# millecker/hadoop-1.0.3-gpu

Hardware: AMD Instinct MI355X
Metric: K-Means job makespan + map-tasks/sec (whole node) at 1/2/4/8 MI355X (higher is better)
Workload: dtype fp32

## Files before the change

### hbmr/models/kmeans.py

```python
from __future__ import annotations

import base64
import logging
import math
import os
import threading
import time

import numpy as np
import torch

from ..gpu.splitjob import SplitJob, SplitSpec
from ..mapred import counters as C

log = logging.getLogger("hbmr.kmeans")

K_KEY = "hbmr.kmeans.k"
D_KEY = "hbmr.kmeans.dims"
INPUT_KEY = "hbmr.kmeans.input"
SPLIT_PTS_KEY = "hbmr.split.points"
CIN_KEY = "hbmr.kmeans.centroids.in"
COUT_KEY = "hbmr.kmeans.centroids.out"
INIT_KEY = "hbmr.kmeans.centroids.init"
NCENTERS_KEY = "hbmr.kmeans.synthetic.centers"
RETURN_KEY = "hbmr.kmeans.return.centroids"
CDIR_KEY = "hbmr.kmeans.centroids.dir"
EXACT_KEY = "hbmr.kmeans.exact"
EXACT_MFMA_KEY = "hbmr.kmeans.exact.mfma"
COMBINER_KEY = "hbmr.kmeans.combiner"
BOUNDS_KEY = "hbmr.kmeans.exact.bounds"

_M32 = 0xFFFFFFFF


def _mix32(x: torch.Tensor) -> torch.Tensor:
    x = x & _M32
    x = ((x ^ (x >> 16)) * 0x45D9F3B) & _M32
    x = ((x ^ (x >> 16)) * 0x45D9F3B) & _M32
    return x ^ (x >> 16)


def _uniform(c: torch.Tensor) -> torch.Tensor:
    return (_mix32(c).to(torch.float64) + 0.5) * (1.0 / 4294967296.0)


def _gauss(c1: torch.Tensor, c2: torch.Tensor) -> torch.Tensor:
    u1 = _uniform(c1)
    u2 = _uniform(c2)
    return torch.sqrt(-2.0 * torch.log(u1)) * torch.cos(2.0 * math.pi * u2)


def synthetic_points(seed: int, start: int, n: int, d: int, centers: int, device,
                     chunk: int = 1 << 18) -> torch.Tensor:
# ... 128 lines not shown
            g[2] += 1
            g[3].append((s, c))
        else:
            loose.append((s, c))
    parts_s, parts_c = [], []
    for bs, bc, n, members in groups.values():
        if n == bs.shape[0] and len({m[0].data_ptr() for m in members}) == n:
            parts_s.append(bs.sum(0))
            parts_c.append(bc.sum(0))
        else:
            loose.extend(members)
    if loose:
        parts_s.append(torch.stack([s for s, _ in loose]).sum(0))
        parts_c.append(torch.stack([c for _, c in loose]).sum(0))
    sums, counts = parts_s[0], parts_c[0]
    for s, c in zip(parts_s[1:], parts_c[1:]):
        sums = sums + s
        counts = counts + c
    return sums, counts


_EXACT_COUNTERS = {"stats": ("EXACT_FLAGGED_POINTS", "EXACT_RELABELLED_POINTS",
                             "EXACT_NEIGHBOUR_SCANS"),
                   "skipped": ("EXACT_BOUND_SKIPPED_POINTS",)}
_EXACT_DEVICE: dict = {}
_EXACT_LOCK = threading.Lock()


def _exact_counter(kind, cin, device):
    key = (kind, cin, str(device))
    with _EXACT_LOCK:
        t = _EXACT_DEVICE.get(key)
        if t is None:
            t = _EXACT_DEVICE[key] = torch.zeros(len(_EXACT_COUNTERS[kind]), dtype=torch.int64,
                                                 device=device)
        return t


def _pop_exact_counters(cin, device):
    got = ((names, _EXACT_DEVICE.pop((kind, cin, str(device)), None))
           for kind, names in _EXACT_COUNTERS.items())
    return [(names, t) for names, t in got if t is not None]

_BASELINES: "dict" = {}
_BASE_LOCK = threading.Lock()
_BASE_MAX = 4096

# ... 96 lines not shown
                    if _BASELINES.get(key) is b:
                        _BASELINES.pop(key)


class KMeansSplitJob(SplitJob):
    collective_reduce = True
    needs_reduce = True

    def configure(self, conf):
        self.conf = conf
        self.k = conf.get_int(K_KEY, 64)
        self.d = conf.get_int(D_KEY, 128)
        self.input = conf.get(INPUT_KEY, "synthetic:100000:1")
        self.split_points = conf.get_int(SPLIT_PTS_KEY, 500_000)
        self.cin = conf.get(CIN_KEY)
        self.cout = conf.get(COUT_KEY)
        self.centers = conf.get_int(NCENTERS_KEY, self.k)
        self.fx_shift = conf.get_int("hbmr.kmeans.fx.shift", 24)
        self.cdir = conf.get(CDIR_KEY)
        self.exact = conf.get_boolean(EXACT_KEY, False)
        self.exact_dtype = torch.bfloat16 if (conf.get(EXACT_MFMA_KEY) or "f16").lower() in (
            "bf16", "bfloat16") else torch.float16
        self.bounds = conf.get_boolean(BOUNDS_KEY, True)
        self.combiner = (conf.get(COMBINER_KEY) or "delta").lower()
        if self.combiner not in ("delta", "sorted"):
            raise ValueError(f"{COMBINER_KEY} must be delta or sorted, not {self.combiner!r}")
        init = conf.get(INIT_KEY)
        if init and self.cin and STORE.host_centroids(self.cin) is None:
            STORE.put_host(self.cin, decode_centroids(init))
        if self.cin and self.cdir and STORE.host_centroids(self.cin) is None:
            path = _centroid_file(self.cdir, self.cin)
            if os.path.exists(path):
                STORE.put_host(self.cin, torch.from_numpy(np.load(path)))

    _split_memo: dict = {}

    def get_splits(self, conf, trackers):
        if self.input.startswith("synthetic:"):
            mk = (self.input, self.split_points, self.d, self.centers, tuple(trackers),
                  self.exact)
            got = KMeansSplitJob._split_memo.get(mk)
            if got is not None:
                return got
            if len(KMeansSplitJob._split_memo) > 16:
                KMeansSplitJob._split_memo.clear()
            out = KMeansSplitJob._split_memo[mk] = self._synthetic_splits(trackers)
# ... 154 lines not shown
                off = 0
                for i in mb.new:
                    n = datas[i].shape[0]
                    mb.install(i, gall[off:off + n])
                    off += n
        return mb.finish()

    def _map_exact(self, ctxs, datas, img, delta):
        from ..ops import kmeans as km
        from ..utils.trace import TRACE
        if TRACE.on:
            TRACE.instant("kmeans.map_exact", n=len(datas))
        ctx = ctxs[0]
        scratch = self._stream_scratch(ctx, "kmeans-exact")
        stats = _exact_counter("stats", self.cin, ctx.device)
        mb = _MapBatch(ctxs, datas, self.k, img, True, delta)
        grown = None
        if mb.have:
            xs = [datas[i] for i in mb.have]
            total = sum(x.shape[0] for x in xs)
            lab = km.scratch_buf(scratch, "labcat", total, torch.int32, ctx.device)
            dws = km.scratch_buf(scratch, "dws", km.delta_workspace_bytes(total, len(xs), self.k),
                                 torch.uint8, ctx.device)
            bounds = skipped = None
            bounded = self.bounds and delta and km.bounds_supported(img)
            if bounded:
                nogap = [b for b in mb.bases if b.gap is None]
                bounds, skipped = mb.bases, _exact_counter("skipped", self.cin, ctx.device)
            km.assign_exact_batch(xs, img, stats, lab, scratch, stream=ctx.stream, bounds=bounds,
                                  skipped=skipped)
            if bounded:
                grown = {id(b): b.gap.numel() * b.gap.element_size() for b in nogap}
            km.delta_combine([x.x32 for x in xs], lab, self.k, *mb.delta_slabs(), dws, mb.bases,
                             fx_shift=img.fx_shift, stream=ctx.stream, keep_bounds=bounded)
            mb.advanced()
        for i in mb.new + mb.plain:
            s, c = mb.out[i]
            s.zero_()
            c.zero_()
            lab = km.map_split_exact(datas[i], img, s, c, scratch, stats, stream=ctx.stream)
            if i in mb.new:
                mb.install(i, lab.clone())
        return mb.finish(grown)

    def map_cpu(self, ctx, points):
        from ..ops import kmeans as km
        cen = STORE.host_centroids(self.cin)
        if cen is None:
            raise KeyError(f"centroids {self.cin!r} not resident")
        sums, counts = km.new_partials(self.k, self.d, "cpu")
        st = [0]
        km.map_split_cpu(points, cen, sums, counts, nthreads=ctx.cpu_threads,
                         fx_shift=self.fx_shift, exact=self.exact, stats=st)
# ... 360 lines not shown
```

### hbmr/ops/_lib.py

```python
from __future__ import annotations

import ctypes
import os
import threading
from pathlib import Path

import torch

_LIB_PATH = Path(__file__).resolve().parent.parent / "lib" / "libhbmr.so"
_lock = threading.Lock()
_lib = None

c_void_p = ctypes.c_void_p
c_long = ctypes.c_long
c_int = ctypes.c_int
c_uint = ctypes.c_uint
c_uint64 = ctypes.c_uint64
c_double_p = ctypes.POINTER(ctypes.c_double)

_SIGS = {
    "hbmr_kmeans_assign_bf16": (c_int, [c_void_p, c_long, c_int, c_void_p, c_void_p, c_int,
                                        c_void_p, c_void_p, c_void_p]),
    "hbmr_kmeans_accum_bf16": (c_int, [c_void_p, c_long, c_int, c_void_p, c_int, c_void_p,
                                       c_void_p, c_int, c_void_p, c_long, c_int, c_void_p]),
    "hbmr_kmeans_accum_f32": (c_int, [c_void_p, c_long, c_int, c_void_p, c_int, c_void_p,
                                      c_void_p, c_int, c_void_p, c_long, c_int, c_void_p]),
    "hbmr_kmeans_assign_top3_bf16": (c_int, [c_void_p, c_long, c_int, c_void_p, c_void_p, c_int,
                                             c_void_p, c_void_p, c_void_p, c_void_p, c_void_p]),
    "hbmr_kmeans_assign_top3_f16": (c_int, [c_void_p, c_long, c_int, c_void_p, c_void_p, c_int,
                                            c_void_p, c_void_p, c_void_p, c_void_p, c_void_p]),
    "hbmr_kmeans_exact_prep": (c_int, [c_void_p, c_long, c_int, c_int, c_int, c_int, c_void_p,
                                       c_void_p, c_void_p, c_void_p, c_void_p]),
    "hbmr_kmeans_assign_top3_q1_grouped": (c_int, [c_int, c_void_p, c_void_p, c_int, c_int,
                                                   c_void_p, c_void_p, c_void_p, c_int, c_void_p,
                                                   c_void_p, c_void_p, c_void_p, c_int, c_int,
                                                   c_void_p, c_void_p, c_void_p, c_void_p,
                                                   c_void_p, c_long, c_void_p, c_void_p]),
    "hbmr_kmeans_bound_workspace_bytes": (c_long, [c_long, c_int, c_int]),
    "hbmr_kmeans_assign_top3_q1_bounded": (c_int, [c_int, c_void_p, c_void_p, c_int, c_int,
                                                   c_void_p, c_void_p, c_int, c_void_p,
                                                   c_void_p, c_void_p, c_void_p, c_int, c_int,
                                                   c_void_p, c_void_p, c_void_p, c_void_p,
                                                   c_void_p, c_long, c_void_p,
                                                   c_void_p, c_void_p, c_void_p, c_void_p,
                                                   c_void_p, c_long, c_void_p, c_void_p]),
    "hbmr_kmeans_centroid_nbr": (c_int, [c_void_p, c_int, c_int, c_int, c_void_p, c_void_p,
                                         c_void_p, c_void_p]),
    "hbmr_kmeans_image16": (c_int, [c_void_p, c_int, c_int, c_int, c_int, c_int, c_void_p,
                                    c_void_p, c_void_p, c_void_p, c_void_p, c_void_p]),
    "hbmr_kmeans_image16_tiled": (c_int, [c_void_p, c_int, c_int, c_void_p, c_void_p]),
    "hbmr_kmeans_set_exact_kernel": (c_int, [c_int]),
    "hbmr_kmeans_get_exact_kernel": (c_int, []),
    "hbmr_kmeans_refine_f32": (c_int, [c_void_p, c_long, c_int, c_int, c_void_p, c_void_p,
                                       c_void_p, c_void_p, c_int, c_int, c_void_p, c_void_p,
                                       c_void_p, c_void_p, c_void_p, c_void_p, c_int, c_void_p,
                                       c_void_p, c_void_p, c_void_p, c_void_p, c_int,
                                       c_void_p]),
    "hbmr_kmeans_refine_batch_bytes": (c_long, [c_int, c_void_p]),
    "hbmr_kmeans_assign_top3_grouped": (c_int, [c_int, c_void_p, c_void_p, c_int, c_int,
                                                c_void_p, c_void_p, c_int, c_void_p, c_void_p,
                                                c_void_p, c_void_p, c_void_p]),
    "hbmr_kmeans_refine_batch_q1g": (c_int, [c_int, c_void_p, c_int, c_int, c_int, c_void_p,
                                             c_void_p, c_void_p, c_void_p, c_void_p, c_void_p,
                                             c_void_p, c_void_p, c_void_p, c_void_p, c_void_p,
                                             c_void_p, c_long, c_void_p, c_void_p]),
    "hbmr_kmeans_refine_batch_q1": (c_int, [c_int, c_void_p, c_int, c_int, c_int, c_int,
                                            c_void_p, c_void_p, c_void_p, c_void_p, c_void_p,
                                            c_void_p, c_void_p, c_void_p, c_void_p, c_void_p,
# ... 229 lines not shown
```

### hbmr/ops/kmeans.py

```python
from __future__ import annotations

import contextlib
import ctypes
import os
import threading

import torch

from . import _lib
from ._lib import ptr
from ..utils.trace import TRACE

SUPPORTED_DP = (64, 128, 256)
FX_SHIFT = 24
NBR_L = 256


def padded_dim(d: int) -> int:
    for dp in SUPPORTED_DP:
        if d <= dp:
            return dp
    raise ValueError(f"feature dim {d} > {SUPPORTED_DP[-1]} not supported by the MFMA kernel")


# ... 407 lines not shown
    _check_refine_dim(img)
    n = split.shape[0]
    dev = split.xb.device
    scratch = {} if scratch is None else scratch
    bufs = scratch.get(("exact", n))
    if bufs is None:
        bufs = scratch[("exact", n)] = tuple(
            torch.empty(m * n, dtype=t, device=dev)
            for m, t in ((1, torch.int32), (2, torch.int32), (1, torch.float32),
                         (2, torch.float32)))
    lab, cand, sc, mg = bufs
    assign_top3(split.xb, img, lab, cand, sc, mg, stream=stream)
    refine_f32(split, img, lab, cand, sc, mg, stats, stream=stream, scratch=scratch)
    return lab


def bounds_supported(img: CentroidImage) -> bool:
    return REFINE_VERSION >= 3 and img.dp <= 128 and GROUPED_EXACT and FUSED_Q1 and \
        img.cen.is_cuda and _lib.load().hbmr_kmeans_get_exact_kernel() == 3


def assign_exact_batch(splits: list, img: CentroidImage, stats: torch.Tensor, out: torch.Tensor,
                       scratch: dict | None = None, stream=None, bounds: list | None = None,
                       skipped: torch.Tensor | None = None) -> None:
    if not splits:
        return
    _check_refine_dim(img)
    if bounds is not None and (len(bounds) != len(splits) or not bounds_supported(img)):
        raise ValueError("bounds: one baseline per split, grouped fused v3 assign (dp <= 128)")
    dev = splits[0].xb.device
    total = sum(sp.shape[0] for sp in splits)
    if out.dtype != torch.int32 or out.numel() < total or not out.is_contiguous():
        raise ValueError("out must be contiguous int32 with room for every split's labels")
    _check_stats(stats)
    dt = splits[0].xb.dtype
    _check_rows([sp.xb for sp in splits], img.dp, (torch.bfloat16, torch.float16))
    if not all(sp.x32.is_contiguous() for sp in splits):
        raise ValueError("exact splits must hold contiguous fp32 rows")
    scratch = {} if scratch is None else scratch
    cand, sc, mg = _top3_scratch(scratch, "exact-batch", max(sp.shape[0] for sp in splits), dev)
    grouped = REFINE_VERSION >= 3 and img.dp <= 128 and GROUPED_EXACT
    with _on(stream):
        c16, ch, *norms = img.image16(dt)
        nbr = (None, None, 0) if grouped else img.neighbors()
        newref = None
        if bounds is not None:
            img.cen.record_stream(torch.cuda.current_stream())
            newref = img.cen.clone()
    lib = _lib.load()
    top3 = lib.hbmr_kmeans_assign_top3_f16 if dt == torch.float16 else \
        lib.hbmr_kmeans_assign_top3_bf16
    st = _lib.stream_handle(stream)
    pc, ps, pm = ptr(cand), ptr(sc), ptr(mg)
    base, off = out.data_ptr(), 0
    for g0 in range(0, len(splits), MAX_REFINE_BATCH):
        group = splits[g0:g0 + MAX_REFINE_BATCH]
        rb = _RefineBatch(group, img, stats, scratch, stream, c16, ch) \
            if REFINE_VERSION >= 3 else None
        if grouped:
            _exact_group(rb, base + 4 * off,
                         None if bounds is None else bounds[g0:g0 + MAX_REFINE_BATCH],
                         skipped, newref)
            off += rb.N
            continue
        if rb is not None:
            rb.open()
        for i, sp in enumerate(group):
            n = sp.shape[0]
            pl = base + 4 * off
            rc = top3(ptr(sp.xb), n, img.dp, ptr(c16), ptr(ch), img.k_pad, pl, pc, ps, pm, st)
            _lib.check(rc, "hbmr_kmeans_assign_top3")
            if rb is not None:
                rb.q1(i, pl, cand, sc, mg)
            else:
                _refine_single(lib, sp, img, norms, nbr, pl, pc, ps, pm, stats, st)
            off += n
        if rb is not None:
            rb.finish()


def order_after(bases: list, attrs: tuple, st) -> None:
    events, blocks = {}, {}
    for b in bases:
        if b.event is not None and b.stream is not None and b.stream != st:
            events[id(b.event)] = b.event
        for a in attrs:
            t = getattr(b, a)
            if t is not None:
                base = t._base if t._base is not None else t
                blocks[id(base)] = base
    for ev in events.values():
        st.wait_event(ev)
    for t in blocks.values():
        t.record_stream(st)


def _bounded_group(rb: _RefineBatch, bases, labels_ptr: int, skipped, newref):
    img, lib = rb.img, rb.lib
    cur = torch.cuda.current_stream() if rb.stream is None else rb.stream
    with torch.cuda.stream(cur):
        for b in bases:
            if b.gap is None:
                b.gap, b.ref = torch.empty(b.g.numel(), dtype=torch.float32, device=rb.dev), None
        for b, n in zip(bases, rb.sizes):
            if b.g.numel() != n or b.gap.numel() != n or \
                    (b.ref is not None and (tuple(b.ref.shape) != tuple(img.cen.shape) or
                                            not b.ref.is_contiguous())):
                raise ValueError("bounds: baseline does not match its split / the centroids")
        order_after(bases, ("g", "gap", "ref"), cur)
        need = int(lib.hbmr_kmeans_bound_workspace_bytes(rb.N, rb.B, img.k))
        bws = scratch_buf(rb.scratch, "bound_ws", need, torch.uint8, rb.dev)
    P = ctypes.c_void_p * rb.B
    cn, cmax, ce, cemax = rb.norms
    refs = [b.ref for b in bases]
    for b in bases:
        b.ref = b.pending = None
    rc = lib.hbmr_kmeans_assign_top3_q1_bounded(
        rb.B, rb.xb, rb.ns, img.dp, int(rb.dt == torch.float16), ptr(img.image16_tiled(rb.dt)),
        ptr(rb.ch), img.k_pad, labels_ptr, rb.xnorm, rb.xbn2, rb.xerr, img.d, img.k, ptr(cn),
        ptr(cmax), ptr(ce), ptr(cemax), ptr(rb.ws), rb.ws.numel(), ptr(rb.pd),
        P(*[b.g.data_ptr() for b in bases]), P(*[b.gap.data_ptr() for b in bases]),
        P(*[ptr(r) for r in refs]), ptr(img.cen), ptr(bws), bws.numel(), ptr(skipped), rb.st)
    _lib.check(rc, "hbmr_kmeans_assign_top3_q1_bounded")
    for b in bases:
        b.pending = newref


def _exact_group(rb: _RefineBatch, labels_ptr: int, bases=None, skipped=None, newref=None):
    img, lib, st = rb.img, rb.lib, rb.st
    f16 = int(rb.dt == torch.float16)
    fused = bases is not None or (FUSED_Q1 and img.dp <= 128)
    if not fused:
        cand, sc, mg = _top3_scratch(rb.scratch, "exact-group", rb.N, rb.dev)
        rc = lib.hbmr_kmeans_assign_top3_grouped(
            rb.B, rb.xb, rb.ns, img.dp, f16, ptr(rb.c16), ptr(rb.ch), img.k_pad, labels_ptr,
            ptr(cand), ptr(sc), ptr(mg), st)
        _lib.check(rc, "hbmr_kmeans_assign_top3_grouped")
    rb.open()
    cn, cmax, ce, cemax = rb.norms
    if fused and TRACE.on:
        TRACE.instant("kmeans.top3_launch", n=rb.B)
    if bases is not None:
        _bounded_group(rb, bases, labels_ptr, skipped, newref)
    elif fused:
        rc = lib.hbmr_kmeans_assign_top3_q1_grouped(
            rb.B, rb.xb, rb.ns, img.dp, f16, ptr(rb.c16), ptr(img.image16_tiled(rb.dt)),
            ptr(rb.ch), img.k_pad, labels_ptr, rb.xnorm, rb.xbn2, rb.xerr, img.d, img.k, ptr(cn),
            ptr(cmax), ptr(ce), ptr(cemax), ptr(rb.ws), rb.ws.numel(), ptr(rb.pd), st)
        _lib.check(rc, "hbmr_kmeans_assign_top3_q1_grouped")
    else:
        rc = lib.hbmr_kmeans_refine_batch_q1g(
            rb.B, rb.ns, img.d, img.k, img.k_pad, rb.xnorm, rb.xbn2, rb.xerr, ptr(cn), ptr(cmax),
            ptr(ce), ptr(cemax), labels_ptr, ptr(cand), ptr(sc), ptr(mg), ptr(rb.ws), rb.ws.numel(),
            ptr(rb.pd), st)
        _lib.check(rc, "hbmr_kmeans_refine_batch_q1g")
    rb.labels_at(labels_ptr)
    rb.finish()


def map_split_exact(split: ExactSplit, img: CentroidImage, sums, counts, scratch: dict,
                    stats: torch.Tensor, stream=None) -> torch.Tensor:
    lab = assign_exact(split, img, stats, scratch, stream=stream)
    ws = scratch_buf(scratch, "ws", workspace_bytes(split.shape[0], img.k), torch.uint8,
                     split.xb.device, floor=1 << 20)
    accumulate(split.x32, lab, img.k, sums, counts, fx_shift=img.fx_shift, stream=stream,
               workspace=ws)
# ... 149 lines not shown
```

### native/include/hbmr/hbmr.h

```cpp
#pragma once
#include <stddef.h>
#include <stdint.h>

#ifdef __cplusplus
extern "C" {
#endif

typedef struct ihipStream_t* hbmr_stream_t;

#ifndef HBMR_NO_HIP_DECLS
#include <hip/hip_runtime_api.h>
int hbmr_kmeans_assign_bf16(const void* X, long n, int dp, const void* C, const float* chalf,
                            int k_pad, int32_t* labels, float* scores, hipStream_t st);
int hbmr_kmeans_accum_bf16(const void* X, long n, int dp, const int32_t* labels, int k,
                           long long* sums, long long* counts, int fx_shift, void* ws,
                           long ws_bytes, int mode, hipStream_t st);
int hbmr_kmeans_accum_f32(const float* X, long n, int dp, const int32_t* labels, int k,
                          long long* sums, long long* counts, int fx_shift, void* ws,
                          long ws_bytes, int mode, hipStream_t st);
int hbmr_kmeans_assign_top3_bf16(const void* X, long n, int dp, const void* C, const float* chalf,
                                 int k_pad, int32_t* labels, int32_t* cand, float* scores,
                                 float* margin, hipStream_t st);
int hbmr_kmeans_assign_top3_f16(const void* X, long n, int dp, const void* C, const float* chalf,
                                int k_pad, int32_t* labels, int32_t* cand, float* scores,
// ... 13 lines not shown
                           const float* nbr_dist, int L, int32_t* labels, const int32_t* cand,
                           const float* scores, const float* margin, unsigned long long* stats,
                           int nstats, hipStream_t st);
int hbmr_kmeans_assign_top3_q1_grouped(int nsplit, const void* const* X, const long* n, int dp,
                                       int f16, const void* C, const void* Ct,
                                       const float* chalf, int k_pad,
                                       int32_t* labels, const float* const* xnorm,
                                       const float* const* xbn2, const float* const* xerr,
                                       int d, int k, const float* cnorm, const float* cmax,
                                       const float* cerr, const float* cerrmax, void* ws,
                                       long ws_bytes, const float* dcc, hipStream_t st);
long hbmr_kmeans_bound_workspace_bytes(long total, int nsplit, int k);
int hbmr_kmeans_assign_top3_q1_bounded(int nsplit, const void* const* X, const long* n, int dp,
                                       int f16, const void* Ct, const float* chalf, int k_pad,
                                       int32_t* labels, const float* const* xnorm,
                                       const float* const* xbn2, const float* const* xerr,
                                       int d, int k, const float* cnorm, const float* cmax,
                                       const float* cerr, const float* cerrmax, void* ws,
                                       long ws_bytes, const float* dcc,
                                       const int32_t* const* g, float* const* gap,
                                       const float* const* ref, const float* cen, void* bws,
                                       long bws_bytes, unsigned long long* skipped,
                                       hipStream_t st);
int hbmr_kmeans_assign_top3_grouped(int nsplit, const void* const* X, const long* n, int dp,
                                    int f16, const void* C, const float* chalf, int k_pad,
                                    int32_t* labels, int32_t* cand, float* scores, float* margin,
                                    hipStream_t st);
int hbmr_kmeans_refine_batch_q1g(int nsplit, const long* ns, int d, int k, int k_pad,
                                 const float* const* xnorm, const float* const* xbn2,
                                 const float* const* xerr, const float* cnorm, const float* cmax,
                                 const float* cerr, const float* cerrmax, const int32_t* labels,
                                 const int32_t* cand, const float* scores, const float* margin,
                                 void* ws, long ws_bytes, const float* dcc, hipStream_t st);
long hbmr_kmeans_refine_batch_bytes(int nsplit, const long* ns);
int hbmr_kmeans_refine_batch_q1(int nsplit, const long* ns, int s, int d, int k, int k_pad,
                                const float* xnorm, const float* xbn2, const float* xerr,
                                const float* cnorm, const float* cmax, const float* cerr,
                                const float* cerrmax, const int32_t* labels, const int32_t* cand,
                                const float* scores, const float* margin,
                                unsigned long long* stats, void* ws, long ws_bytes, int reset,
                                const float* dcc, hipStream_t st);
int hbmr_kmeans_refine_batch_finish(int nsplit, const long* ns, const float* const* x32,
                                    int32_t* const* labels, int d, int ldx, const float* C32,
                                    int k, int k_pad, const float* cmax, const float* cerrmax,
                                    const int32_t* nbr_idx, const float* nbr_dist, int L,
                                    unsigned long long* stats, int nstats, void* ws,
// ... 228 lines not shown
```

### native/kernels/kmeans.hip

```cpp
#include "common.h"
#include "../include/hbmr/hbmr.h"
#include <algorithm>
#include <cstdlib>
#include <cstring>
#include <type_traits>
#include "kmeans/assign.h"
#include "kmeans/grouped.h"
#include "kmeans/combine.h"
#include "kmeans/refine.h"
#include "kmeans/image.h"
#include "kmeans/refine_queue.h"
#include "kmeans/fused.h"
#include "kmeans/bounded.h"
#include "kmeans/launch.h"

extern "C" {

int hbmr_kmeans_assign_bf16(const void* X, long n, int dp, const void* C, const float* chalf,
                            int k_pad, int32_t* labels, float* scores, hipStream_t st) {
  return dispatch_dp(dp, [&](auto D) {
    return launch_assign<D()>(X, n, C, chalf, k_pad, labels, scores, st);
  });
}

// ... 191 lines not shown
  if (exact_kernel() == 3) {
    if (!Ct) return (int)hipErrorInvalidValue;
    const auto [kern, lds] = fused_kernel(dp, f16, [](auto D, auto F) {
      return &kmeans_assign_top3_q1_v3_kernel<D(), F()>;
    });
    hipLaunchKernelGGL(kern, dim3((unsigned)nb), dim3(256), lds, st, t,
                       reinterpret_cast<const __bf16*>(Ct), chalf, k_pad / 32, labels, fin);
    return (int)hipGetLastError();
  }
  const auto [kern, lds] = fused_kernel(dp, f16, [](auto D, auto F) {
    return &kmeans_assign_top3_q1_grouped_kernel<D(), F()>;
  });
  hipLaunchKernelGGL(kern, dim3((unsigned)nb), dim3(AssignV2<64>::THREADS), lds, st, t,
                     reinterpret_cast<const __bf16*>(C), chalf, k_pad / 32, labels, fin);
  return (int)hipGetLastError();
}

long hbmr_kmeans_bound_workspace_bytes(long total, int nsplit, int k) {
  if (total < 0 || nsplit <= 0 || nsplit > kMaxGroup || k <= 0) return -1;
  const size_t sh = ((size_t)nsplit * k * sizeof(float) + 255) & ~(size_t)255;
  return (long)(kBoundHdr + sh + (size_t)total * sizeof(uint32_t));
}

int hbmr_kmeans_assign_top3_q1_bounded(int nsplit, const void* const* X, const long* n, int dp,
                                       int f16, const void* Ct, const float* chalf, int k_pad,
                                       int32_t* labels, const float* const* xnorm,
                                       const float* const* xbn2, const float* const* xerr,
                                       int d, int k, const float* cnorm, const float* cmax,
                                       const float* cerr, const float* cerrmax, void* ws,
                                       long ws_bytes, const float* dcc,
                                       const int32_t* const* g, float* const* gap,
                                       const float* const* ref, const float* cen, void* bws,
                                       long bws_bytes, unsigned long long* skipped,
                                       hipStream_t st) {
  if (nsplit <= 0 || nsplit > kMaxGroup || k_pad % 32 || k <= 0 || k_pad < k || d <= 0 ||
      d > kRefineMaxDp || !labels || ((uintptr_t)ws & 255) || (dp != 64 && dp != 128) || !Ct ||
      !g || !gap || !ref || !cen || !bws || ((uintptr_t)bws & 255))
    return (int)hipErrorInvalidValue;
  TopQ1Table t;
  SweepTable sw;
  GapTable gt;
  ShiftTable sh;
  memset(&t, 0, sizeof(t));
  memset(&sw, 0, sizeof(sw));
  memset(&gt, 0, sizeof(gt));
  memset(&sh, 0, sizeof(sh));
  t.nsplit = sw.nsplit = nsplit;
  long total = 0, nb = 0, nsb = 0;
  int nref = 0;
  for (int i = 0; i < nsplit; ++i) {
    if (n[i] < 0 || n[i] > 0x7fffffffL || (n[i] > 0 && (!gap[i] || (ref[i] && !g[i]))))
      return (int)hipErrorInvalidValue;
    fill_topq1(t, i, X, xnorm, xbn2, xerr, total, nb);
    sw.off[i] = total;
    sw.blk[i] = nsb;
    sw.n[i] = n[i];
    sw.g[i] = g[i];
    gt.gap[i] = gap[i];
    if (ref[i]) {
      int r = 0;
      while (r < nref && sh.ref[r] != ref[i]) ++r;
      if (r == nref) sh.ref[nref++] = ref[i];
      sw.rid[i] = r;
      sw.gap[i] = gap[i];
    }
    total += n[i];
    nb += ceil_div(n[i], kFusedPts);
    nsb += ceil_div(n[i], 256 * kSweepPer);
  }
  t.off[nsplit] = total;
  t.blk[nsplit] = nb;
  sw.blk[nsplit] = nsb;
  const RefineLayout Ly = refine_layout(nsplit, n);
  if (ws_bytes < (long)Ly.bytes ||
      bws_bytes < hbmr_kmeans_bound_workspace_bytes(total, nsplit, k))
    return (int)hipErrorInvalidValue;
  char* w = static_cast<char*>(ws);
  char* bw = static_cast<char*>(bws);
  HBMR_RETURN_IF_ERROR(hipMemsetAsync(w, 0, kHdrClear, st));
  if (nb == 0) return 0;
  if (nb > 0x7fffffffL) return (int)hipErrorInvalidValue;
  HBMR_RETURN_IF_ERROR(hipMemsetAsync(bw, 0, kBoundHdr, st));
  uint32_t* cnt = reinterpret_cast<uint32_t*>(bw);
  uint32_t* smax = cnt + kMaxGroup;
  float* shift = reinterpret_cast<float*>(bw + kBoundHdr);
  uint32_t* idx = reinterpret_cast<uint32_t*>(
      bw + kBoundHdr + (((size_t)nsplit * k * sizeof(float) + 255) & ~(size_t)255));
  if (nref > 0) {
    hipLaunchKernelGGL(kmeans_bound_shift_kernel, dim3((unsigned)k, (unsigned)nref), dim3(64), 0,
                       st, sh, cen, k, d, shift, smax);
    HBMR_RETURN_IF_ERROR(hipGetLastError());
  }
  hipLaunchKernelGGL(kmeans_bound_sweep_kernel, dim3((unsigned)nsb), dim3(256), 0, st, sw, k,
                     shift, reinterpret_cast<const float*>(smax), labels, cnt, idx);
  HBMR_RETURN_IF_ERROR(hipGetLastError());
  const FusedQ1Fin fin = make_fused_fin(k, d, k_pad, cnorm, cerr, dcc, cmax, cerrmax, w, Ly);
  const auto [kern, lds] = fused_kernel(dp, f16, [](auto D, auto F) {
    return &kmeans_assign_top3_q1_bounded_kernel<D(), F()>;
  });
  hipLaunchKernelGGL(kern, dim3((unsigned)nb), dim3(256), lds, st, t, gt,
                     reinterpret_cast<const __bf16*>(Ct), chalf, k_pad / 32, labels, fin,
                     (const uint32_t*)cnt, (const uint32_t*)idx, skipped);
  return (int)hipGetLastError();
}

int hbmr_kmeans_refine_f32(const float* X32, long n, int d, int ldx, const float* xnorm,
                           const float* xbn2, const float* xerr, const float* C32, int k,
                           int k_pad, const float* cnorm, const float* cmax, const float* cerr,
                           const float* cerrmax, const int32_t* nbr_idx,
                           const float* nbr_dist, int L, int32_t* labels, const int32_t* cand,
                           const float* scores, const float* margin, unsigned long long* stats,
                           int nstats, hipStream_t st) {
  if (n <= 0) return 0;
  if (d > ldx || d > kRefineMaxDp || k <= 0 || k_pad < k || L < 1 || L > k)
    return (int)hipErrorInvalidValue;
  const double pack_rel = pack_rel_of(k_pad);
  const long blocks = (n + 255) / 256;
  const bool v2_ok = d % 8 == 0 && ldx % 4 == 0 && ((uintptr_t)X32 & 15) == 0 &&
                     ((uintptr_t)C32 & 15) == 0;
  if (v2_ok) {
    auto kern = d <= 128 ? kmeans_refine_v2_kernel<1> : kmeans_refine_v2_kernel<2>;
    hipLaunchKernelGGL(kern, dim3((unsigned)blocks), dim3(256), 0, st, X32, n, d, ldx, xnorm,
                       xbn2, xerr, C32, k, cnorm, cmax, cerr, cerrmax, pack_rel, nbr_idx,
                       nbr_dist, L, labels, cand, scores, margin, stats, nstats);
    return (int)hipGetLastError();
  }
// ... 187 lines not shown
```

### native/kernels/kmeans/bounded.h

```cpp
#pragma once
#include "../common.h"
#include "fused.h"

namespace {

constexpr int kSweepPer = 8;
constexpr int kBoundHdr = 512;

struct ShiftTable {
  const float* ref[kMaxGroup];
};

__global__ __launch_bounds__(64) void kmeans_bound_shift_kernel(
    const ShiftTable tbl, const float* __restrict__ cen, int k, int d, float* __restrict__ shift,
    uint32_t* __restrict__ smax) {
  const int j = blockIdx.x, r = blockIdx.y;
  const float* a = cen + (size_t)j * d;
  const float* b = tbl.ref[r] + (size_t)j * d;
  double acc = 0.0;
  for (int i = threadIdx.x; i < d; i += 64) {
    const double e = (double)a[i] - (double)b[i];
    acc = fma(e, e, acc);
  }
#pragma unroll
// ... 75 lines not shown
      for (int i = 0; i < kSweepPer; ++i) {
        const uint32_t c = wcnt[w][i];
        wcnt[w][i] = tot;
        tot += c;
      }
    base_s = tot ? atomicAdd(cnt + s, tot) : 0u;
  }
  __syncthreads();
  uint32_t* out = idx + o + base_s;
#pragma unroll
  for (int i = 0; i < kSweepPer; ++i)
    if (list[i]) out[wcnt[wave][i] + rank[i]] = (uint32_t)(p0 + i * 256 + tid);
}

struct GapTable {
  float* gap[kMaxGroup];
};

template <int D, bool F16>
__global__ __launch_bounds__(256, kExactMinB) void kmeans_assign_top3_q1_bounded_kernel(
    const TopQ1Table tbl, const GapTable gt, const __bf16* __restrict__ Ct,
    const float* __restrict__ chalf, int ntiles, int32_t* __restrict__ labels, FusedQ1Fin fin,
    const uint32_t* __restrict__ cnt, const uint32_t* __restrict__ idx,
    unsigned long long* __restrict__ skipped) {
  extern __shared__ __attribute__((aligned(16))) char smem[];
  if (blockIdx.x == 0 && threadIdx.x == 0 && skipped != nullptr) {
    unsigned long long sk = 0;
    for (int i = 0; i < tbl.nsplit; ++i)
      sk += (unsigned long long)(tbl.off[i + 1] - tbl.off[i]) - cnt[i];
    if (sk) atomicAdd(skipped, sk);
  }
  const long b = hbmr_xcd_remap(blockIdx.x, gridDim.x);
  int lo = 0, hi = tbl.nsplit;
  while (hi - lo > 1) {
    const int mid = (lo + hi) >> 1;
    if (tbl.blk[mid] <= b) lo = mid; else hi = mid;
  }
  const int s = __builtin_amdgcn_readfirstlane(lo);
  const long nl = (long)__builtin_amdgcn_readfirstlane(cnt[s]);
  const long lb = b - tbl.blk[s];
  if (lb * 256 >= nl) return;
  const long o = tbl.off[s];
  fin.xnorm = tbl.xnorm[s];
  fin.xbn2 = tbl.xbn2[s];
  fin.xerr = tbl.xerr[s];
  fin.sidx = s;
  fin.idx = idx + o;
  fin.gap = gt.gap[s];
  assign_tile_v3<D, F16, true>(tbl.X[s], nl, Ct, chalf, ntiles, labels + o, lb, smem, fin);
}


}
```

Baseline: 10180.

## Add neighbour-scan pre-pass to settle bound-failing points before fused MFMA assign

Adds an intermediate kernel between the bound sweep and the fused top-3 MFMA assignment. For each point that failed the drift bound, it computes exact fp32 distances to its previous centroid and a few nearby centroids taken from the centroid neighbour table. If the winner is provably separated, it writes the label and a fresh gap directly and leaves the point out of the compacted list. Only the remaining points go to the full assign kernel, which cuts full-K MFMA work at the cost of an extra launch, a memset, per-point gathers and a compaction.

```diff
diff --git a/hbmr/models/kmeans.py b/hbmr/models/kmeans.py
--- a/hbmr/models/kmeans.py
+++ b/hbmr/models/kmeans.py
@@ -29,6 +29,7 @@
 EXACT_MFMA_KEY = "hbmr.kmeans.exact.mfma"
 COMBINER_KEY = "hbmr.kmeans.combiner"
 BOUNDS_KEY = "hbmr.kmeans.exact.bounds"
+BOUNDS_SCAN_KEY = "hbmr.kmeans.exact.bounds.scan"
 
 _M32 = 0xFFFFFFFF
 
@@ -203,7 +204,8 @@
 
 _EXACT_COUNTERS = {"stats": ("EXACT_FLAGGED_POINTS", "EXACT_RELABELLED_POINTS",
                              "EXACT_NEIGHBOUR_SCANS"),
-                   "skipped": ("EXACT_BOUND_SKIPPED_POINTS",)}
+                   "skipped": ("EXACT_BOUND_SKIPPED_POINTS",),
+                   "scan": ("EXACT_BOUND_SCAN_POINTS",)}
 _EXACT_DEVICE: dict = {}
 _EXACT_LOCK = threading.Lock()
 
@@ -346,6 +348,7 @@
         self.exact_dtype = torch.bfloat16 if (conf.get(EXACT_MFMA_KEY) or "f16").lower() in (
             "bf16", "bfloat16") else torch.float16
         self.bounds = conf.get_boolean(BOUNDS_KEY, True)
+        self.bounds_scan = conf.get_boolean(BOUNDS_SCAN_KEY, True)
         self.combiner = (conf.get(COMBINER_KEY) or "delta").lower()
         if self.combiner not in ("delta", "sorted"):
             raise ValueError(f"{COMBINER_KEY} must be delta or sorted, not {self.combiner!r}")
@@ -546,13 +549,15 @@
             lab = km.scratch_buf(scratch, "labcat", total, torch.int32, ctx.device)
             dws = km.scratch_buf(scratch, "dws", km.delta_workspace_bytes(total, len(xs), self.k),
                                  torch.uint8, ctx.device)
-            bounds = skipped = None
+            bounds = skipped = settled = None
             bounded = self.bounds and delta and km.bounds_supported(img)
             if bounded:
                 nogap = [b for b in mb.bases if b.gap is None]
                 bounds, skipped = mb.bases, _exact_counter("skipped", self.cin, ctx.device)
+                if self.bounds_scan:
+                    settled = _exact_counter("scan", self.cin, ctx.device)
             km.assign_exact_batch(xs, img, stats, lab, scratch, stream=ctx.stream, bounds=bounds,
-                                  skipped=skipped)
+                                  skipped=skipped, scan=self.bounds_scan, settled=settled)
             if bounded:
                 grown = {id(b): b.gap.numel() * b.gap.element_size() for b in nogap}
             km.delta_combine([x.x32 for x in xs], lab, self.k, *mb.delta_slabs(), dws, mb.bases,
diff --git a/hbmr/ops/_lib.py b/hbmr/ops/_lib.py
--- a/hbmr/ops/_lib.py
+++ b/hbmr/ops/_lib.py
@@ -44,6 +44,16 @@
                                                    c_void_p, c_long, c_void_p,
                                                    c_void_p, c_void_p, c_void_p, c_void_p,
                                                    c_void_p, c_long, c_void_p, c_void_p]),
+    "hbmr_kmeans_bound_scan_workspace_bytes": (c_long, [c_long, c_int, c_int]),
+    "hbmr_kmeans_assign_top3_q1_bounded_scan": (c_int, [c_int, c_void_p, c_void_p, c_int, c_int,
+                                                        c_void_p, c_void_p, c_int, c_void_p,
+                                                        c_void_p, c_void_p, c_void_p, c_int, c_int,
+                                                        c_void_p, c_void_p, c_void_p, c_void_p,
+                                                        c_void_p, c_long, c_void_p,
+                                                        c_void_p, c_void_p, c_void_p, c_void_p,
+                                                        c_void_p, c_long, c_void_p,
+                                                        c_void_p, c_int, c_void_p, c_void_p, c_int,
+                                                        c_void_p, c_void_p]),
     "hbmr_kmeans_centroid_nbr": (c_int, [c_void_p, c_int, c_int, c_int, c_void_p, c_void_p,
                                          c_void_p, c_void_p]),
     "hbmr_kmeans_image16": (c_int, [c_void_p, c_int, c_int, c_int, c_int, c_int, c_void_p,
diff --git a/hbmr/ops/kmeans.py b/hbmr/ops/kmeans.py
--- a/hbmr/ops/kmeans.py
+++ b/hbmr/ops/kmeans.py
@@ -453,7 +453,8 @@
 
 def assign_exact_batch(splits: list, img: CentroidImage, stats: torch.Tensor, out: torch.Tensor,
                        scratch: dict | None = None, stream=None, bounds: list | None = None,
-                       skipped: torch.Tensor | None = None) -> None:
+                       skipped: torch.Tensor | None = None, scan: bool = False,
+                       settled: torch.Tensor | None = None) -> None:
     if not splits:
         return
     _check_refine_dim(img)
@@ -491,7 +492,7 @@
         if grouped:
             _exact_group(rb, base + 4 * off,
                          None if bounds is None else bounds[g0:g0 + MAX_REFINE_BATCH],
-                         skipped, newref)
+                         skipped, newref, scan, settled)
             off += rb.N
             continue
         if rb is not None:
@@ -526,7 +527,8 @@
         t.record_stream(st)
 
 
-def _bounded_group(rb: _RefineBatch, bases, labels_ptr: int, skipped, newref):
+def _bounded_group(rb: _RefineBatch, bases, labels_ptr: int, skipped, newref, scan=False,
+                   settled=None):
     img, lib = rb.img, rb.lib
     cur = torch.cuda.current_stream() if rb.stream is None else rb.stream
     with torch.cuda.stream(cur):
@@ -539,25 +541,36 @@
                                             not b.ref.is_contiguous())):
                 raise ValueError("bounds: baseline does not match its split / the centroids")
         order_after(bases, ("g", "gap", "ref"), cur)
-        need = int(lib.hbmr_kmeans_bound_workspace_bytes(rb.N, rb.B, img.k))
-        bws = scratch_buf(rb.scratch, "bound_ws", need, torch.uint8, rb.dev)
+        scan = scan and img.d % 8 == 0 and rb.nbr is not None
+        size = lib.hbmr_kmeans_bound_scan_workspace_bytes if scan else \
+            lib.hbmr_kmeans_bound_workspace_bytes
+        bws = scratch_buf(rb.scratch, "bound_ws", int(size(rb.N, rb.B, img.k)), torch.uint8,
+                          rb.dev)
     P = ctypes.c_void_p * rb.B
     cn, cmax, ce, cemax = rb.norms
     refs = [b.ref for b in bases]
     for b in bases:
         b.ref = b.pending = None
-    rc = lib.hbmr_kmeans_assign_top3_q1_bounded(
-        rb.B, rb.xb, rb.ns, img.dp, int(rb.dt == torch.float16), ptr(img.image16_tiled(rb.dt)),
-        ptr(rb.ch), img.k_pad, labels_ptr, rb.xnorm, rb.xbn2, rb.xerr, img.d, img.k, ptr(cn),
-        ptr(cmax), ptr(ce), ptr(cemax), ptr(rb.ws), rb.ws.numel(), ptr(rb.pd),
-        P(*[b.g.data_ptr() for b in bases]), P(*[b.gap.data_ptr() for b in bases]),
-        P(*[ptr(r) for r in refs]), ptr(img.cen), ptr(bws), bws.numel(), ptr(skipped), rb.st)
-    _lib.check(rc, "hbmr_kmeans_assign_top3_q1_bounded")
+    args = (rb.B, rb.xb, rb.ns, img.dp, int(rb.dt == torch.float16),
+            ptr(img.image16_tiled(rb.dt)), ptr(rb.ch), img.k_pad, labels_ptr, rb.xnorm, rb.xbn2,
+            rb.xerr, img.d, img.k, ptr(cn), ptr(cmax), ptr(ce), ptr(cemax), ptr(rb.ws),
+            rb.ws.numel(), ptr(rb.pd), P(*[b.g.data_ptr() for b in bases]),
+            P(*[b.gap.data_ptr() for b in bases]), P(*[ptr(r) for r in refs]), ptr(img.cen),
+            ptr(bws), bws.numel(), ptr(skipped))
+    if scan:
+        ni, nd, L = rb.nbr
+        rc = lib.hbmr_kmeans_assign_top3_q1_bounded_scan(
+            *args, rb.x32, rb.splits[0].x32.shape[1], ptr(ni), ptr(nd), L, ptr(settled), rb.st)
+        _lib.check(rc, "hbmr_kmeans_assign_top3_q1_bounded_scan")
+    else:
+        rc = lib.hbmr_kmeans_assign_top3_q1_bounded(*args, rb.st)
+        _lib.check(rc, "hbmr_kmeans_assign_top3_q1_bounded")
     for b in bases:
         b.pending = newref
 
 
-def _exact_group(rb: _RefineBatch, labels_ptr: int, bases=None, skipped=None, newref=None):
+def _exact_group(rb: _RefineBatch, labels_ptr: int, bases=None, skipped=None, newref=None,
+                 scan=False, settled=None):
     img, lib, st = rb.img, rb.lib, rb.st
     f16 = int(rb.dt == torch.float16)
     fused = bases is not None or (FUSED_Q1 and img.dp <= 128)
@@ -572,7 +585,7 @@
     if fused and TRACE.on:
         TRACE.instant("kmeans.top3_launch", n=rb.B)
     if bases is not None:
-        _bounded_group(rb, bases, labels_ptr, skipped, newref)
+        _bounded_group(rb, bases, labels_ptr, skipped, newref, scan, settled)
     elif fused:
         rc = lib.hbmr_kmeans_assign_top3_q1_grouped(
             rb.B, rb.xb, rb.ns, img.dp, f16, ptr(rb.c16), ptr(img.image16_tiled(rb.dt)),
diff --git a/native/include/hbmr/hbmr.h b/native/include/hbmr/hbmr.h
--- a/native/include/hbmr/hbmr.h
+++ b/native/include/hbmr/hbmr.h
@@ -59,6 +59,16 @@
                                        const float* const* ref, const float* cen, void* bws,
                                        long bws_bytes, unsigned long long* skipped,
                                        hipStream_t st);
+long hbmr_kmeans_bound_scan_workspace_bytes(long total, int nsplit, int k);
+int hbmr_kmeans_assign_top3_q1_bounded_scan(
+    int nsplit, const void* const* X, const long* n, int dp, int f16, const void* Ct,
+    const float* chalf, int k_pad, int32_t* labels, const float* const* xnorm,
+    const float* const* xbn2, const float* const* xerr, int d, int k, const float* cnorm,
+    const float* cmax, const float* cerr, const float* cerrmax, void* ws, long ws_bytes,
+    const float* dcc, const int32_t* const* g, float* const* gap, const float* const* ref,
+    const float* cen, void* bws, long bws_bytes, unsigned long long* skipped,
+    const float* const* x32, int ldx, const int32_t* nbr_idx, const float* nbr_dist, int L,
+    unsigned long long* settled, hipStream_t st);
 int hbmr_kmeans_assign_top3_grouped(int nsplit, const void* const* X, const long* n, int dp,
                                     int f16, const void* C, const float* chalf, int k_pad,
                                     int32_t* labels, int32_t* cand, float* scores, float* margin,
diff --git a/native/kernels/kmeans.hip b/native/kernels/kmeans.hip
--- a/native/kernels/kmeans.hip
+++ b/native/kernels/kmeans.hip
@@ -237,30 +237,50 @@
   return (long)(kBoundHdr + sh + (size_t)total * sizeof(uint32_t));
 }
 
-int hbmr_kmeans_assign_top3_q1_bounded(int nsplit, const void* const* X, const long* n, int dp,
-                                       int f16, const void* Ct, const float* chalf, int k_pad,
-                                       int32_t* labels, const float* const* xnorm,
-                                       const float* const* xbn2, const float* const* xerr,
-                                       int d, int k, const float* cnorm, const float* cmax,
-                                       const float* cerr, const float* cerrmax, void* ws,
-                                       long ws_bytes, const float* dcc,
-                                       const int32_t* const* g, float* const* gap,
-                                       const float* const* ref, const float* cen, void* bws,
-                                       long bws_bytes, unsigned long long* skipped,
-                                       hipStream_t st) {
+long hbmr_kmeans_bound_scan_workspace_bytes(long total, int nsplit, int k) {
+  const long base = hbmr_kmeans_bound_workspace_bytes(total, nsplit, k);
+  if (base < 0) return -1;
+  return (long)((((size_t)base + 255) & ~(size_t)255) + kScanHdr +
+                (size_t)total * sizeof(uint32_t));
+}
+
+struct BoundScanArgs {
+  const float* const* x32;
+  int ldx;
+  const int32_t* nbr_idx;
+  const float* nbr_dist;
+  int L;
+  unsigned long long* settled;
+};
+
+static int bounded_pass(int nsplit, const void* const* X, const long* n, int dp, int f16,
+                        const void* Ct, const float* chalf, int k_pad, int32_t* labels,
+                        const float* const* xnorm, const float* const* xbn2,
+                        const float* const* xerr, int d, int k, const float* cnorm,
+                        const float* cmax, const float* cerr, const float* cerrmax, void* ws,
+                        long ws_bytes, const float* dcc, const int32_t* const* g,
+                        float* const* gap, const float* const* ref, const float* cen, void* bws,
+                        long bws_bytes, unsigned long long* skipped, const BoundScanArgs* sc,
+                        hipStream_t st) {
   if (nsplit <= 0 || nsplit > kMaxGroup || k_pad % 32 || k <= 0 || k_pad < k || d <= 0 ||
       d > kRefineMaxDp || !labels || ((uintptr_t)ws & 255) || (dp != 64 && dp != 128) || !Ct ||
       !g || !gap || !ref || !cen || !bws || ((uintptr_t)bws & 255))
+    return (int)hipErrorInvalidValue;
+  if (sc && (!sc->x32 || !sc->nbr_idx || !sc->nbr_dist || sc->L < 1 || sc->L > k ||
+             sc->ldx < d))
     return (int)hipErrorInvalidValue;
   TopQ1Table t;
   SweepTable sw;
   GapTable gt;
   ShiftTable sh;
+  ScanTable scan;
   memset(&t, 0, sizeof(t));
   memset(&sw, 0, sizeof(sw));
   memset(&gt, 0, sizeof(gt));
   memset(&sh, 0, sizeof(sh));
-  t.nsplit = sw.nsplit = nsplit;
+  memset(&scan, 0, sizeof(scan));
+  t.nsplit = sw.nsplit = scan.nsplit = nsplit;
+  bool scan_ok = sc && d % 8 == 0 && sc->ldx % 4 == 0 && ((uintptr_t)cen & 15) == 0;
   long total = 0, nb = 0, nsb = 0;
   int nref = 0;
   for (int i = 0; i < nsplit; ++i) {
@@ -279,6 +299,14 @@
       sw.rid[i] = r;
       sw.gap[i] = gap[i];
     }
+    if (sc) {
+      if (n[i] > 0 && !sc->x32[i]) return (int)hipErrorInvalidValue;
+      scan_ok = scan_ok && ((uintptr_t)sc->x32[i] & 15) == 0;
+      scan.x32[i] = sc->x32[i];
+      scan.g[i] = sw.g[i];
+      scan.gap[i] = sw.gap[i];
+      scan.off[i] = total;
+    }
     total += n[i];
     nb += ceil_div(n[i], kFusedPts);
     nsb += ceil_div(n[i], 256 * kSweepPer);
@@ -287,8 +315,9 @@
   t.blk[nsplit] = nb;
   sw.blk[nsplit] = nsb;
   const RefineLayout Ly = refine_layout(nsplit, n);
+  const long base_bytes = hbmr_kmeans_bound_workspace_bytes(total, nsplit, k);
   if (ws_bytes < (long)Ly.bytes ||
-      bws_bytes < hbmr_kmeans_bound_workspace_bytes(total, nsplit, k))
+      bws_bytes < (sc ? hbmr_kmeans_bound_scan_workspace_bytes(total, nsplit, k) : base_bytes))
     return (int)hipErrorInvalidValue;
   char* w = static_cast<char*>(ws);
   char* bw = static_cast<char*>(bws);
@@ -309,14 +338,62 @@
   hipLaunchKernelGGL(kmeans_bound_sweep_kernel, dim3((unsigned)nsb), dim3(256), 0, st, sw, k,
                      shift, reinterpret_cast<const float*>(smax), labels, cnt, idx);
   HBMR_RETURN_IF_ERROR(hipGetLastError());
+  const uint32_t* lcnt = cnt;
+  const uint32_t* lidx = idx;
+  if (scan_ok) {
+    char* sb = bw + (((size_t)base_bytes + 255) & ~(size_t)255);
+    uint32_t* cnt2 = reinterpret_cast<uint32_t*>(sb);
+    uint32_t* idx2 = reinterpret_cast<uint32_t*>(sb + kScanHdr);
+    HBMR_RETURN_IF_ERROR(hipMemsetAsync(cnt2, 0, kScanHdr, st));
+    const unsigned gs =
+        (unsigned)std::max<long>(1, std::min<long>(kRefineGrid, ceil_div(total, kScanPerBlk)));
+    auto kern = d <= 128 ? kmeans_bound_scan_kernel<1> : kmeans_bound_scan_kernel<2>;
+    hipLaunchKernelGGL(kern, dim3(gs), dim3(256), 0, st, scan, d, sc->ldx, cen, k, sc->nbr_idx,
+                       sc->nbr_dist, sc->L, labels, (const uint32_t*)cnt, (const uint32_t*)idx,
+                       cnt2, idx2, sc->settled);
+    HBMR_RETURN_IF_ERROR(hipGetLastError());
+    lcnt = cnt2;
+    lidx = idx2;
+  }
   const FusedQ1Fin fin = make_fused_fin(k, d, k_pad, cnorm, cerr, dcc, cmax, cerrmax, w, Ly);
   const auto [kern, lds] = fused_kernel(dp, f16, [](auto D, auto F) {
     return &kmeans_assign_top3_q1_bounded_kernel<D(), F()>;
   });
   hipLaunchKernelGGL(kern, dim3((unsigned)nb), dim3(256), lds, st, t, gt,
-                     reinterpret_cast<const __bf16*>(Ct), chalf, k_pad / 32, labels, fin,
-                     (const uint32_t*)cnt, (const uint32_t*)idx, skipped);
-  return (int)hipGetLastError();
+                     reinterpret_cast<const __bf16*>(Ct), chalf, k_pad / 32, labels, fin, lcnt,
+                     lidx, (const uint32_t*)cnt, skipped);
+  return (int)hipGetLastError();
+}
+
+int hbmr_kmeans_assign_top3_q1_bounded(int nsplit, const void* const* X, const long* n, int dp,
+                                       int f16, const void* Ct, const float* chalf, int k_pad,
+                                       int32_t* labels, const float* const* xnorm,
+                                       const float* const* xbn2, const float* const* xerr,
+                                       int d, int k, const float* cnorm, const float* cmax,
+                                       const float* cerr, const float* cerrmax, void* ws,
+                                       long ws_bytes, const float* dcc,
+                                       const int32_t* const* g, float* const* gap,
+                                       const float* const* ref, const float* cen, void* bws,
+                                       long bws_bytes, unsigned long long* skipped,
+                                       hipStream_t st) {
+  return bounded_pass(nsplit, X, n, dp, f16, Ct, chalf, k_pad, labels, xnorm, xbn2, xerr, d, k,
+                      cnorm, cmax, cerr, cerrmax, ws, ws_bytes, dcc, g, gap, ref, cen, bws,
+                      bws_bytes, skipped, nullptr, st);
+}
+
+int hbmr_kmeans_assign_top3_q1_bounded_scan(
+    int nsplit, const void* const* X, const long* n, int dp, int f16, const void* Ct,
+    const float* chalf, int k_pad, int32_t* labels, const float* const* xnorm,
+    const float* const* xbn2, const float* const* xerr, int d, int k, const float* cnorm,
+    const float* cmax, const float* cerr, const float* cerrmax, void* ws, long ws_bytes,
+    const float* dcc, const int32_t* const* g, float* const* gap, const float* const* ref,
+    const float* cen, void* bws, long bws_bytes, unsigned long long* skipped,
+    const float* const* x32, int ldx, const int32_t* nbr_idx, const float* nbr_dist, int L,
+    unsigned long long* settled, hipStream_t st) {
+  const BoundScanArgs sc{x32, ldx, nbr_idx, nbr_dist, L, settled};
+  return bounded_pass(nsplit, X, n, dp, f16, Ct, chalf, k_pad, labels, xnorm, xbn2, xerr, d, k,
+                      cnorm, cmax, cerr, cerrmax, ws, ws_bytes, dcc, g, gap, ref, cen, bws,
+                      bws_bytes, skipped, &sc, st);
 }
 
 int hbmr_kmeans_refine_f32(const float* X32, long n, int d, int ldx, const float* xnorm,
diff --git a/native/kernels/kmeans/bounded.h b/native/kernels/kmeans/bounded.h
--- a/native/kernels/kmeans/bounded.h
+++ b/native/kernels/kmeans/bounded.h
@@ -121,12 +121,12 @@
     const TopQ1Table tbl, const GapTable gt, const __bf16* __restrict__ Ct,
     const float* __restrict__ chalf, int ntiles, int32_t* __restrict__ labels, FusedQ1Fin fin,
     const uint32_t* __restrict__ cnt, const uint32_t* __restrict__ idx,
-    unsigned long long* __restrict__ skipped) {
+    const uint32_t* __restrict__ swept, unsigned long long* __restrict__ skipped) {
   extern __shared__ __attribute__((aligned(16))) char smem[];
   if (blockIdx.x == 0 && threadIdx.x == 0 && skipped != nullptr) {
     unsigned long long sk = 0;
     for (int i = 0; i < tbl.nsplit; ++i)
-      sk += (unsigned long long)(tbl.off[i + 1] - tbl.off[i]) - cnt[i];
+      sk += (unsigned long long)(tbl.off[i + 1] - tbl.off[i]) - swept[i];
     if (sk) atomicAdd(skipped, sk);
   }
   const long b = hbmr_xcd_remap(blockIdx.x, gridDim.x);
@@ -149,5 +149,201 @@
   assign_tile_v3<D, F16, true>(tbl.X[s], nl, Ct, chalf, ntiles, labels + o, lb, smem, fin);
 }
 
-
-}
+constexpr int kScanM = 3;
+constexpr int kScanNbr = kScanM + 2;
+constexpr int kScanPerBlk = 4 * kQ2Per;
+constexpr int kScanBuf = 256;
+constexpr int kScanHdr = 256;
+
+struct ScanTable {
+  int nsplit;
+  const float* x32[kMaxGroup];
+  const int32_t* g[kMaxGroup];
+  float* gap[kMaxGroup];
+  long off[kMaxGroup];
+};
+
+struct ScanItem {
+  uint32_t row;
+  int32_t split, g;
+};
+
+template <int NM>
+__global__ __launch_bounds__(256) void kmeans_bound_scan_kernel(
+    const ScanTable tbl, int d, int ldx, const float* __restrict__ C32, int k,
+    const int32_t* __restrict__ nbr_idx, const float* __restrict__ nbr_dist, int L,
+    int32_t* __restrict__ labels, const uint32_t* __restrict__ cnt,
+    const uint32_t* __restrict__ idx, uint32_t* __restrict__ cnt2, uint32_t* __restrict__ idx2,
+    unsigned long long* __restrict__ settled) {
+  const int tid = threadIdx.x, lane = tid & 63, wave = tid >> 6;
+  const int grp = lane / kQ2Lanes, sub = lane % kQ2Lanes;
+  __shared__ uint32_t pre[kMaxGroup + 1];
+  __shared__ uint2 sbuf[kScanBuf];
+  __shared__ uint32_t scnt[kMaxGroup], sbase[kMaxGroup];
+  __shared__ uint32_t wc[2][4];
+  __shared__ uint32_t nset;
+  if (tid == 0) {
+    uint32_t acc = 0;
+    for (int i = 0; i < tbl.nsplit; ++i) {
+      pre[i] = acc;
+      acc += cnt[i];
+    }
+    pre[tbl.nsplit] = acc;
+    nset = 0;
+  }
+  if (tid < kMaxGroup) scnt[tid] = 0;
+  __syncthreads();
+  const uint32_t total = pre[tbl.nsplit];
+  const uint32_t stride = gridDim.x * kScanPerBlk;
+  const uint32_t off = wave * kQ2Per + grp;
+  auto fetch = [&](uint32_t i) {
+    int lo = 0, hi = tbl.nsplit;
+    while (hi - lo > 1) {
+      const int mid = (lo + hi) >> 1;
+      if (pre[mid] <= i) lo = mid; else hi = mid;
+    }
+    ScanItem q;
+    q.split = lo;
+    q.row = idx[tbl.off[lo] + (i - pre[lo])];
+    q.g = tbl.gap[lo] != nullptr ? tbl.g[lo][q.row] : -1;
+    return q;
+  };
+  auto flush = [&](uint32_t m) {
+    __syncthreads();
+    uint2 o = make_uint2(0u, 0u);
+    uint32_t r = 0;
+    if ((uint32_t)tid < m) {
+      o = sbuf[tid];
+      r = atomicAdd(&scnt[o.x], 1u);
+    }
+    __syncthreads();
+    if (tid < kMaxGroup && scnt[tid]) sbase[tid] = atomicAdd(cnt2 + tid, scnt[tid]);
+    __syncthreads();
+    if ((uint32_t)tid < m) idx2[tbl.off[o.x] + sbase[o.x] + r] = o.y;
+    if (tid < kMaxGroup) scnt[tid] = 0;
+    __syncthreads();
+  };
+  const double rel = (double)(16 * NM + 8) * 0x1p-24 * 1.01, aeps = 0x1p-120;
+  const int ne = L < kScanNbr ? L : kScanNbr;
+  uint32_t mine = 0;
+  uint32_t fill = 0;
+  int par = 0;
+  uint32_t bb = blockIdx.x * kScanPerBlk;
+  ScanItem e;
+  if (bb < total) e = fetch(min(bb + off, total - 1));
+  for (; bb < total; bb += stride) {
+    const ScanItem q = e;
+    const bool have = bb + off < total;
+    const uint32_t nb = bb + stride;
+    if (nb < total) e = fetch(min(nb + off, total - 1));
+    const bool direct = (uint32_t)q.g >= (uint32_t)k;
+    const int g = direct ? 0 : q.g;
+    float xf[16 * NM];
+    float fg;
+    int32_t ni;
+    float nd;
+    {
+      float cg[16 * NM];
+      load_row16<NM>(tbl.x32[q.split] + (size_t)q.row * ldx, d, sub, xf);
+      load_row16<NM>(C32 + (size_t)g * d, d, sub, cg);
+      const size_t at = (size_t)g * L + (sub < ne ? sub : ne - 1);
+      ni = nbr_idx[at];
+      nd = nbr_dist[at];
+      fg = 0.f;
+#pragma unroll
+      for (int i = 0; i < 16 * NM; ++i) {
+        const float t = xf[i] - cg[i];
+        fg = fmaf(t, t, fg);
+      }
+      fg = row_sum8f(fg);
+    }
+    const double r0_hi = sqrt((double)fg * (1.0 + rel) + aeps) * (1.0 + 0x1p-40);
+    const double lim = 2.0 * r0_hi * (1.0 + 0x1p-20);
+    const bool other = sub < ne && ni != g;
+    const bool inside = other && (double)nd <= lim;
+    const bool past = other && (double)nd > lim;
+    const uint32_t qm = (uint32_t)(__ballot(inside) >> (grp * kQ2Lanes)) & 0xffu;
+    const uint32_t pm = (uint32_t)(__ballot(past) >> (grp * kQ2Lanes)) & 0xffu;
+    const bool start = !direct && __popc(qm) <= kScanM && pm != 0u;
+    const float nd_next = __shfl(nd, grp * kQ2Lanes + (pm ? __ffs(pm) - 1 : 0));
+    int cj[kScanM];
+    bool cv[kScanM];
+    {
+      uint32_t mm = qm;
+#pragma unroll
+      for (int v = 0; v < kScanM; ++v) {
+        cv[v] = mm != 0u;
+        const int c = __shfl(ni, grp * kQ2Lanes + (cv[v] ? __ffs(mm) - 1 : 0));
+        cj[v] = cv[v] ? c : g;
+        mm &= mm - 1u;
+      }
+    }
+    float f[kScanM];
+    {
+      float cr[kScanM][16 * NM];
+#pragma unroll
+      for (int v = 0; v < kScanM; ++v) load_row16<NM>(C32 + (size_t)cj[v] * d, d, sub, cr[v]);
+#pragma unroll
+      for (int v = 0; v < kScanM; ++v) f[v] = 0.f;
+#pragma unroll
+      for (int i = 0; i < 16 * NM; ++i) {
+#pragma unroll
+        for (int v = 0; v < kScanM; ++v) {
+          const float t = xf[i] - cr[v][i];
+          f[v] = fmaf(t, t, f[v]);
+        }
+      }
+#pragma unroll
+      for (int v = 0; v < kScanM; ++v) f[v] = row_sum8f(f[v]);
+    }
+    int w = g;
+    double dw = fg;
+#pragma unroll
+    for (int v = 0; v < kScanM; ++v)
+      if (cv[v] && (double)f[v] < dw) { w = cj[v]; dw = f[v]; }
+    const double whi = dw * (1.0 + rel) + aeps;
+    auto beats = [&](double dj) { return dj * (1.0 - rel) - aeps > whi; };
+    bool sep = isfinite(whi) && (w == g || beats(fg));
+#pragma unroll
+    for (int v = 0; v < kScanM; ++v) sep = sep && (!cv[v] || w == cj[v] || beats(f[v]));
+    const bool settle = have && start && sep;
+    if (settle && sub == 0) {
+      auto lower = [&](double dj) {
+        return sqrt(fmax(0.0, dj * (1.0 - rel) - aeps)) * (1.0 - 0x1p-40);
+      };
+      double lo = (double)nd_next - r0_hi;
+      if (w != g) lo = fmin(lo, lower(fg));
+#pragma unroll
+      for (int v = 0; v < kScanM; ++v)
+        if (cv[v] && cj[v] != w) lo = fmin(lo, lower(f[v]));
+      const double gv = (lo - sqrt(whi) * (1.0 + 0x1p-40)) * (1.0 - 0x1p-30);
+      labels[tbl.off[q.split] + q.row] = w;
+      tbl.gap[q.split][q.row] = fmaxf(0.f, __double2float_rd(gv));
+      ++mine;
+    }
+    const bool spill = have && sub == 0 && !settle;
+    const unsigned long long m = __ballot(spill);
+    if (lane == 0) wc[par][wave] = (uint32_t)__popcll(m);
+    __syncthreads();
+    uint32_t before = 0, all = 0;
+#pragma unroll
+    for (int v = 0; v < 4; ++v) {
+      const uint32_t c = wc[par][v];
+      before += v < wave ? c : 0u;
+      all += c;
+    }
+    if (spill) sbuf[fill + before + lane_rank(m)] = make_uint2((uint32_t)q.split, q.row);
+    fill += all;
+    par ^= 1;
+    if (fill > kScanBuf - kScanPerBlk) {
+      flush(fill);
+      fill = 0;
+    }
+  }
+  if (fill) flush(fill);
+  if (mine) atomicAdd(&nset, mine);
+  __syncthreads();
+  if (tid == 0 && nset && settled != nullptr) atomicAdd(settled, (unsigned long long)nset);
+}
+
+}
```

After: 9849. -3.2%, worse.
